# freudh/lbt

Hardware: AMD Instinct MI355X
Metric: train-step samples/sec, ResNet-20 CIFAR-10 8-bit DFP, 1/2/4/8 MI355X (higher is better)
Workload: dtype int8; 1 GPU; ResNet-20 CIFAR-10 8-bit DFXP W/A/G train step (fwd+bwd+SGD-momentum+range update); global_batch=128, per_gpu_batch=128, parallelism=dp1, hip_graph=True, executor=fused, grad_range=-6, loss_diverged=False

## Files before the change

### include/lbt_dfxp.h

```cpp
#ifndef LBT_DFXP_H
#define LBT_DFXP_H

#include <stdint.h>

#ifdef __cplusplus
extern "C" {
#endif

#define LBT_OK 0
#define LBT_EINVAL 1001

#define LBT_NSHARD 32
#define LBT_CSTRIDE 32

enum {
  LBT_OUT_I8 = 0,
  LBT_OUT_U8OFF = 1,
  LBT_OUT_I16 = 2,
  LBT_OUT_F32 = 3
};

typedef struct lbt_qdesc {
  const int32_t* exps;
  int32_t* counts;
// ... 191 lines not shown
                             lbt_qdesc qw, const int8_t* gq2, const int8_t* wd2, int32_t ksd2,
                             lbt_conv_desc d2, lbt_qdesc qg2, lbt_qdesc qw2, int32_t w4,
                             const lbt_chain_bwd_a* a, void* stream);
int lbt_conv_dgrad_chain_i8w4(const int8_t* gq, const uint8_t* wd4, int32_t ksd, lbt_conv_desc d, lbt_qdesc qg,
                              lbt_qdesc qw, const float* add_src, const lbt_chain_bwd_a* a, void* stream);
int lbt_conv_dgrad_chain_wgrad_i8(const int8_t* gq, const int8_t* wd, int32_t ksd, lbt_conv_desc d, lbt_qdesc qg,
                                  lbt_qdesc qw, const float* add_src, const lbt_chain_bwd_a* a, const int8_t* xq,
                                  int32_t x_u8off, int32_t* slab, int32_t nsplit, int32_t nshard, void* stream);
int lbt_conv_dgrad_chain_wgrad_i8w4(const int8_t* gq, const uint8_t* wd4, int32_t ksd, lbt_conv_desc d,
                                    lbt_qdesc qg, lbt_qdesc qw, const float* add_src, const lbt_chain_bwd_a* a,
                                    const int8_t* xq, int32_t x_u8off, int32_t* slab, int32_t nsplit,
                                    int32_t nshard, void* stream);

typedef struct lbt_chain_bwd_b {
  const int8_t* G; lbt_qdesc qng; const int8_t* qn_codes; lbt_qdesc qn; const float* ms;
  const int64_t* sums; int64_t n;
  float* dx; int8_t* gq; lbt_qdesc qo; int64_t* gcolsum;
  int64_t rows, inner; int32_t C;
} lbt_chain_bwd_b;
int lbt_bn_chain_bwd_b(const lbt_chain_bwd_b* a, void* stream);
int lbt_conv_stem_bwd(const lbt_chain_bwd_b* b, const int16_t* x, lbt_conv_desc d, int32_t* slab, int32_t nshard,
                      void* stream);
int lbt_bn_chain_bwd_b_pair(const lbt_chain_bwd_b* a, const lbt_chain_bwd_b* b, void* stream);

typedef struct lbt_wgrad_job {
  const int8_t* xq; int32_t x_u8off; const int8_t* gq; lbt_conv_desc d;
  int32_t* slab; int32_t nsplit, nshard;
} lbt_wgrad_job;

int lbt_conv_wgrad_many_i8(const lbt_wgrad_job* jobs, int32_t njobs, void* stream);
int lbt_conv_wgrad_many_stem_i8(const lbt_wgrad_job* jobs, int32_t njobs, const lbt_chain_bwd_b* b, const int16_t* x,
                                lbt_conv_desc d, int32_t* slab, int32_t nshard, void* stream);

typedef struct lbt_conv_bwd {
  lbt_chain_bwd_b b;
  const int8_t* wd; int32_t ksd; int32_t w4; lbt_conv_desc d; lbt_qdesc qw;
  const float* add_src;
  lbt_chain_bwd_a a;
  lbt_wgrad_job w;
} lbt_conv_bwd;
int lbt_conv_bwd_fused_i8(const lbt_conv_bwd* p, void* stream);

typedef struct lbt_conv_bwd2 {
  lbt_chain_bwd_b b1, bs;
  const int8_t* wd1; int32_t ksd1; const int8_t* wds; int32_t ksds; int32_t w4;
  lbt_conv_desc d1, ds; lbt_qdesc qw1, qws;
  lbt_chain_bwd_a a;
} lbt_conv_bwd2;
int lbt_conv_bwd2_fused_i8(const lbt_conv_bwd2* p, void* stream);

typedef struct lbt_conv_fwd {
  lbt_chain_fwd c;
  const int8_t* wf; int32_t ksf; int32_t w4; const int32_t* wcolsum; lbt_conv_desc d; lbt_qdesc qw;
  int8_t* yq; lbt_qdesc qout; int64_t* ychsum;
} lbt_conv_fwd;
int lbt_conv_fwd_fused_i8(const lbt_conv_fwd* p, void* stream);

int lbt_conv_fused_tile_rows(int32_t Cin, int64_t N, int32_t H);

int lbt_bn_bwd_a_wide(const float* g, lbt_qdesc qrg, const int8_t* R, const float* gamma_q, lbt_qdesc qng,
                      const int8_t* qn, int16_t* gout, float* dout, int64_t* sums, int64_t rows, int64_t inner,
                      int32_t C, void* stream);
int lbt_bn_bwd_b_wide(const int16_t* G, lbt_qdesc qng, const int8_t* qn, lbt_qdesc qn_q, const float* ms,
                      const int64_t* sums, int64_t n, float* dx, int64_t rows, int32_t C, void* stream);

int lbt_bn_bwd_a_wide_masked(const float* g, const float* g2, const float* y_mask, const uint8_t* y_bits,
// ... 176 lines not shown
```

### lbt_amd/_lib.py

```python
import ctypes
import os

import torch

HERE = os.path.dirname(os.path.abspath(__file__))
LIB_PATH = os.environ.get("LBT_LIBRARY") or os.path.join(HERE, "liblbt_dfxp.so")

NSHARD = 32
STEM_WG_PIXELS = 256
CSTRIDE = 32
OUT_I8, OUT_U8OFF, OUT_I16, OUT_F32 = 0, 1, 2, 3
ABI_VERSION = 22

c_void_p, c_int32, c_int64, c_uint32, c_uint64, c_float = (
    ctypes.c_void_p, ctypes.c_int32, ctypes.c_int64, ctypes.c_uint32, ctypes.c_uint64, ctypes.c_float)


class QDesc(ctypes.Structure):
    _fields_ = [("exps", c_void_p), ("counts", c_void_p), ("step", c_void_p), ("seed", c_uint64),
                ("qid", c_uint32), ("slot", c_int32), ("bits", c_int32), ("stochastic", c_int32),
                ("noise", c_void_p)]


NO_Q = QDesc()


class ConvDesc(ctypes.Structure):
    _fields_ = [(n, c_int32) for n in ("N", "H", "W", "Cin", "Cout", "KH", "KW", "SH", "SW",
                                       "PT", "PB", "PL", "PR", "Ho", "Wo")]


class BnNorm(ctypes.Structure):
    _fields_ = [("q", c_void_p), ("qn", QDesc), ("chsum", c_void_p), ("n", c_int64),
                ("eps", c_float), ("momentum", c_float), ("one_minus_momentum", c_float),
                ("ms", c_void_p), ("run_mean", c_void_p), ("run_var", c_void_p), ("frozen", c_int32),
                ("ms_in", c_int32)]


class ChainBranch(ctypes.Structure):
    _fields_ = [("nrm", BnNorm), ("xin", c_void_p), ("qr", QDesc), ("rout", c_void_p), ("gb", c_void_p)]


class ChainFwd(ctypes.Structure):
    _fields_ = [("b1", ChainBranch), ("b2", ChainBranch), ("has_b2", c_int32),
                ("res", c_void_p), ("relu", c_int32), ("y", c_void_p),
# ... 141 lines not shown
    "lbt_dfxp_counts_fold": [_P, c_int32, _P, _P],
    "lbt_dfxp_range_update_folded": [_P, _P, _P, _P, _P, c_int32, _P, _P],
    "lbt_dfxp_quantize_weight": [_P, c_int32, c_int32, c_int32, c_int32, QDesc, _P, _P, c_int32, _P, c_int32,
                                 _P, _P],
    "lbt_conv_fwd_i8": [_P, c_int32, _P, c_int32, _P, ConvDesc, QDesc, QDesc, _P, _P, QDesc, _P, _P],
    "lbt_conv_dgrad_i8": [_P, _P, c_int32, ConvDesc, QDesc, QDesc, _P, _P, _P],
    "lbt_conv_fwd_i8w4": [_P, c_int32, _P, c_int32, _P, ConvDesc, QDesc, QDesc, _P, _P, QDesc, _P, _P],
    "lbt_conv_dgrad_i8w4": [_P, _P, c_int32, ConvDesc, QDesc, QDesc, _P, _P, _P],
    "lbt_pack_int4": [_P, _P, c_int64, _P],
    "lbt_conv_fwd_igemm": [_P, c_int32, _P, c_int32, _P, ConvDesc, QDesc, QDesc, _P, _P],
    "lbt_conv_dgrad_igemm": [_P, c_int32, _P, c_int32, ConvDesc, QDesc, QDesc, _P, _P, _P],
    "lbt_conv_wgrad_igemm": [_P, _P, c_int32, ConvDesc, _P, c_int32, c_int32, _P],
    "lbt_igemm_workspace_bytes": [ConvDesc, c_int32, c_int32],
    "lbt_igemm_get_tuning": [_P],
    "lbt_igemm_set_tuning": [_P],
    "lbt_conv_fwd_igemm_q": [_P, c_int32, _P, c_int32, ConvDesc, QDesc, QDesc, _P, QDesc, _P, _P],
    "lbt_conv_fwd_igemm_ws": [_P, c_int32, _P, c_int32, _P, ConvDesc, QDesc, QDesc, _P, _P, c_int64, _P],
    "lbt_conv_dgrad_igemm_ws": [_P, c_int32, _P, c_int32, ConvDesc, QDesc, QDesc, _P, _P, _P, c_int64, _P],
    "lbt_conv_dgrad_igemm_bna": [_P, _P, c_int32, ConvDesc, QDesc, QDesc, ctypes.POINTER(DgradBna), _P, _P, c_int64,
                                 _P],
    "lbt_bn_moments": [ctypes.POINTER(BnNorm), c_int32, _P],
    "lbt_conv_dgrad_igemm_bn3": [_P, _P, c_int32, ConvDesc, QDesc, QDesc, ctypes.POINTER(DgradBn3), _P, _P, c_int64,
                                 _P],
    "lbt_conv_wgrad_igemm_store": [_P, _P, c_int32, ConvDesc, _P, c_int32, _P],
    "lbt_conv_dgrad_chain_i8w4": [_P, _P, c_int32, ConvDesc, QDesc, QDesc, _P, _P, _P],
    "lbt_conv_dgrad_chain_i8": [_P, _P, c_int32, ConvDesc, QDesc, QDesc, _P, _P, _P],
    "lbt_conv_dgrad_chain_wgrad_i8": [_P, _P, c_int32, ConvDesc, QDesc, QDesc, _P, _P, _P, c_int32, _P, c_int32,
                                      c_int32, _P],
    "lbt_conv_dgrad_chain_wgrad_i8w4": [_P, _P, c_int32, ConvDesc, QDesc, QDesc, _P, _P, _P, c_int32, _P, c_int32,
                                        c_int32, _P],
    "lbt_conv_wgrad_i8": [_P, c_int32, _P, ConvDesc, _P, c_int32, c_int32, _P],
    "lbt_conv_wgrad_many_i8": [_P, c_int32, _P],
    "lbt_conv_wgrad_many_stem_i8": [_P, c_int32, _P, _P, ConvDesc, _P, c_int32, _P],
    "lbt_conv_wgrad_reduce": [_P, c_int32, c_int32, c_int32, c_int32, _P, QDesc, QDesc, _P, c_float, _P, _P],
    "lbt_conv_fwd_generic": [_P, c_int32, _P, ConvDesc, QDesc, QDesc, _P, _P],
    "lbt_conv_dgrad_generic": [_P, _P, ConvDesc, QDesc, QDesc, _P, _P, _P],
    "lbt_conv_wgrad_generic": [_P, c_int32, _P, ConvDesc, _P, c_int32, _P],
    "lbt_conv_dgrad_generic16": [_P, _P, ConvDesc, QDesc, QDesc, _P, _P, _P],
    "lbt_conv_wgrad_generic16": [_P, c_int32, _P, ConvDesc, _P, c_int32, _P],
    "lbt_conv_wgrad_reduce64": [_P, c_int32, c_int32, c_int32, QDesc, QDesc, _P, c_float, _P, _P],
    "lbt_conv_wgrad_reduce64_many": [_P, c_int32, c_int32, _P],
    "lbt_conv_stem_fwd": [_P, _P, ConvDesc, QDesc, QDesc, _P, _P, QDesc, _P, _P],
    "lbt_conv_stem_wgrad": [_P, _P, ConvDesc, _P, c_int32, _P],
    "lbt_conv_stem_bwd": [_P, _P, ConvDesc, _P, c_int32, _P],
    "lbt_conv_bwd2_fused_i8": [_P, _P],
    "lbt_conv_fwd2_fused_i8": [_P, _P],
    "lbt_conv_wgrad_reduce_x": [_P, c_int32, c_int32, c_int32, c_int32, _P, _P, _P],
    "lbt_conv_wgrad_reduce64_x": [_P, c_int32, c_int32, c_int32, _P, _P],
    "lbt_dense_wgrad_x": [_P, _P, c_int32, c_int32, c_int32, c_int32, _P, _P],
    "lbt_bn_param_grads_x": [_P, c_int32, _P, _P, _P],
    "lbt_softmax_xent_n": [_P, _P, c_int32, c_int32, c_int32, _P, _P, _P, _P],
    "lbt_softmax_xent_wide_n": [_P, _P, c_int32, c_int32, c_int32, _P, _P, _P, _P],
    "lbt_conv_stem_wide_fwd": [_P, _P, ConvDesc, QDesc, QDesc, _P, _P],
    "lbt_stem_wide_nsplit": [ConvDesc],
    "lbt_conv_stem_wide_wgrad": [_P, c_int32, _P, c_int32, ConvDesc, _P, c_int32, _P],
    "lbt_dense_pack": [_P, c_int32, c_int32, _P, c_int32, _P, c_int32, _P],
    "lbt_flat_weight_blocks": [c_int64],
    "lbt_dfxp_quantize_weights_flat": [_P, _P, c_int32, c_int32, _P],
    "lbt_bn_bwd_a_wide_masked": [_P, _P, _P, _P, c_int32, QDesc, _P, _P, QDesc, _P, QDesc, _P, _P, _P, _P, c_int64, c_int64,
                                 c_int32, _P],
    "lbt_bn_bwd_b_wide_q": [_P, QDesc, _P, QDesc, _P, _P, c_int64, _P, QDesc, c_int64, c_int64, c_int32, _P],
    "lbt_dense_gemm": [_P, c_int32, c_int32, c_int32, _P, c_int32, c_int32, c_int32, QDesc, QDesc, _P, _P],
    "lbt_dense_wgrad": [_P, _P, c_int32, c_int32, c_int32, c_int32, QDesc, QDesc, _P, c_float, _P, _P],
    "lbt_softmax_xent_wide": [_P, _P, c_int32, c_int32, _P, _P, _P],
    "lbt_bn_chain_fwd": [_P, _P],
    "lbt_bn_chain_bwd_a": [_P, _P],
# ... 96 lines not shown
```

### lbt_amd/csrc/conv_mfma.hip

```cpp
#include "conv_epilogue.h"
#include "chain_flags.h"
#include "conv_wgrad_body.h"
#include "lds_tr.h"
#include "stem_bwd.h"

using namespace lbt;

namespace {

constexpr int kThreads = 256;

enum { MODE_FWD = 0, MODE_DGRAD = 1 };

struct GemmArgs {
  const int8_t* a;
  const int8_t* b;
  int ks;
  int nslices;
  int a_fill;
  const int32_t* colsum;
  lbt_conv_desc d;
  lbt_qdesc qa, qb;
  float* y;
  const float* add_src;
  int8_t* yq;
  lbt_qdesc qout;
  int64_t* ychsum;
  int64_t M;
  int ncol;
  lbt_chain_bwd_a chain;
};

template <int MODE, int CS, int NT, int CF, int NB, bool W4, bool DUAL = false>
__device__ __forceinline__ void conv_gemm_body(const GemmArgs& p, uint32_t bid, const GemmArgs* p2 = nullptr) {
  using G = EpiGeom<NT>;
  constexpr int NTW = G::NTW, WPM = G::WPM, MTB = G::MTB;
  __shared__ EpiShared<NT> sh;
// ... 530 lines not shown
                                             lbt_qdesc qg, lbt_qdesc qw, const float* add_src,
                                             const lbt_chain_bwd_a* a, const int8_t* xq, int32_t x_u8off,
                                             int32_t* slab, int32_t nsplit, int32_t nshard, void* stream) {
  return dgrad_chain_wgrad<false>(gq, wd, ksd, d, qg, qw, add_src, a, xq, x_u8off, slab, nsplit, nshard, stream);
}
extern "C" int lbt_conv_dgrad_chain_wgrad_i8w4(const int8_t* gq, const uint8_t* wd4, int32_t ksd, lbt_conv_desc d,
                                               lbt_qdesc qg, lbt_qdesc qw, const float* add_src,
                                               const lbt_chain_bwd_a* a, const int8_t* xq, int32_t x_u8off,
                                               int32_t* slab, int32_t nsplit, int32_t nshard, void* stream) {
  if (qw.bits > 4) return LBT_EINVAL;
  return dgrad_chain_wgrad<true>(gq, (const int8_t*)wd4, ksd, d, qg, qw, add_src, a, xq, x_u8off, slab, nsplit,
                                 nshard, stream);
}

extern "C" int lbt_conv_wgrad_i8(const int8_t* xq, int32_t x_u8off, const int8_t* gq, lbt_conv_desc d,
                                    int32_t* slab, int32_t nsplit, int32_t nshard, void* stream) {
  WgradArgs wa;
  uint32_t blocks = 0;
  const int e = wgrad_setup(xq, x_u8off, gq, d, slab, nsplit, nshard, wa, blocks);
  if (e) return e;
  hipStream_t st = (hipStream_t)stream;
  switch (d.Cin / 16) {
    case 1: hipLaunchKernelGGL(conv_wgrad_kernel<1>, dim3(blocks), dim3(kThreads), 0, st, wa); break;
    case 2: hipLaunchKernelGGL(conv_wgrad_kernel<2>, dim3(blocks), dim3(kThreads), 0, st, wa); break;
    case 4: hipLaunchKernelGGL(conv_wgrad_kernel<4>, dim3(blocks), dim3(kThreads), 0, st, wa); break;
    case 8: hipLaunchKernelGGL(conv_wgrad_kernel<8>, dim3(blocks), dim3(kThreads), 0, st, wa); break;
    default: return LBT_EINVAL;
  }
  return (int)hipGetLastError();
}

namespace {
constexpr int kMaxWJobs = 24;
#ifndef LBT_WGM_OCC
#define LBT_WGM_OCC 4
#endif
#ifndef LBT_WGM_BUFS
#define LBT_WGM_BUFS 2
#endif
#ifndef LBT_WGX
#define LBT_WGX 0
#endif
constexpr int kWgmBufs = LBT_WGM_BUFS;
constexpr int kFW = 8;
constexpr int kHaloMax = 3;
struct WgradMany {
  WgradArgs j[kMaxWJobs];
  uint32_t start[kMaxWJobs + 1];
  int32_t fast[kMaxWJobs];
  int n;
};
union WgradManyShared {
  WgradShared<1, kFW> s1;
  WgradShared<2, kFW> s2;
  int8_t stage[kFW][5 * 1024];
  int red[kFW / 2][9 * 256];
};

bool wgrad_s1_ok(const lbt_conv_desc& d, int nsplit) {
  if (d.KH != 3 || d.KW != 3 || d.SH != 1 || d.SW != 1 || d.PT != 1 || d.PB != 1 || d.PL != 1 || d.PR != 1 ||
      d.Ho != d.H || d.Wo != d.W || d.W > 64 || 64 % d.W || d.H % (64 / d.W) ||
      (64 / d.W + 2) * (d.W + 2) > 64 * kHaloMax)
    return false;
  const int64_t chunks = (int64_t)d.N * d.H * d.W / 64;
  return nsplit > 0 && chunks % nsplit == 0;
}

LBT_DEV v4i tr_frag_at(const int8_t* img, int oa, int ob) {
  typedef __attribute__((address_space(3))) v2i lds_v2i;
  const v2i lo = __builtin_amdgcn_ds_read_tr8_b64_v2i32((lds_v2i*)(img + oa));
  const v2i hi = __builtin_amdgcn_ds_read_tr8_b64_v2i32((lds_v2i*)(img + ob));
  return v4i{lo.x, lo.y, hi.x, hi.y};
}

__device__ __forceinline__ void wgrad_s1_body(const WgradArgs& wa, uint32_t bid, WgradManyShared& sm) {
  const lbt_conv_desc& d = wa.d;
  const int H = d.H, W = d.W, Cin = d.Cin, Cout = d.Cout;
  const int ncs = Cin >> 4, ncos = Cout >> 4, nsplit = wa.nsplit;
  const int total = nsplit * ncs * ncos;
  const int xchunk = (total + 7) >> 3;
  const int u = (int)(bid & 7) * xchunk + (int)(bid >> 3);
  if (u >= total) return;
  const int split = u / (ncs * ncos), urem = u - split * (ncs * ncos);
  const int cis = urem / ncos, cos = urem - cis * ncos;
  const int lane = threadIdx.x & 63, wave = wave_id();
  const int j = lane & 15, kg = lane >> 4;
  const int RB = 64 / W, Wp = W + 2, nhalo = (RB + 2) * Wp;
  const int64_t cps = (int64_t)d.N * H * W / 64 / nsplit;
  const int64_t c0 = (int64_t)split * cps;
  const int nmine = cps > wave ? (int)((cps - wave + kFW - 1) / kFW) : 0;
  const int HW = H * W;
  const int fill = wa.x_fill;
  int8_t* st = sm.stage[wave];
  int8_t* gs = st + 4096;
  const int pa = 16 * kg + (j >> 1), pb = pa + 8;
  const int oxa = ((pa / W) * Wp + pa % W) * 16 + 8 * (j & 1);
  const int oxb = ((pb / W) * Wp + pb % W) * 16 + 8 * (j & 1);
  const int oga = pa * 16 + 8 * (j & 1), ogb = pb * 16 + 8 * (j & 1);
  int hoff[kHaloMax];
  uint32_t hin = 0, htop = 0, hbot = 0;
#pragma unroll
  for (int i = 0; i < kHaloMax; ++i) {
    const int t = lane + 64 * i;
    const int hy = t / Wp, hx = t - hy * Wp;
    hoff[i] = ((hy - 1) * W + hx - 1) * Cin;
    hin |= (uint32_t)(t < nhalo && hx >= 1 && hx <= W) << i;
    htop |= (uint32_t)(hy == 0) << i;
    hbot |= (uint32_t)(hy == RB + 1) << i;
  }

  struct Buf {
    v4i x[kHaloMax], g;
    uint32_t valid;
  };
  auto load = [&](Buf& b, int64_t c) {
    const int64_t p0 = c * 64;
    const int n = (int)(p0 / HW), row0 = (int)(p0 - (int64_t)n * HW) / W;
    const int8_t* xim = wa.xq + (p0 * Cin + cis * 16);
    b.valid = hin & ~(row0 == 0 ? htop : 0u) & ~(row0 + RB == H ? hbot : 0u);
#pragma unroll
    for (int i = 0; i < kHaloMax; ++i)
      b.x[i] = *reinterpret_cast<const v4i*>(xim + ((b.valid >> i) & 1 ? hoff[i] : 0));
    b.g = *reinterpret_cast<const v4i*>(wa.gq + (p0 + lane) * Cout + cos * 16);
  };
  v4i acc[9];
#pragma unroll
  for (int t = 0; t < 9; ++t) acc[t] = v4i{0, 0, 0, 0};
  auto cidx = [&](int s) { return c0 + wave + (int64_t)(s < nmine ? s : nmine - 1) * kFW; };
  auto step = [&](Buf& b, int s) {
    if constexpr (!(LBT_WGX & 2)) {
#pragma unroll
      for (int i = 0; i < kHaloMax; ++i) {
        const int t = lane + 64 * i;
        const v4i v = (b.valid >> i) & 1 ? b.x[i] : v4i{fill, fill, fill, fill};
        if (t < nhalo) *reinterpret_cast<v4i*>(st + t * 16) = v;
      }
      *reinterpret_cast<v4i*>(gs + lane * 16) = s < nmine ? b.g : v4i{0, 0, 0, 0};
    }
    asm volatile("" ::: "memory");
    if constexpr (!(LBT_WGX & 1)) load(b, cidx(s + kWgmBufs));
    const v4i bfrag = (LBT_WGX & 4) ? b.g : tr_frag_at(gs, oga, ogb);
#pragma unroll
    for (int t = 0; t < 9; ++t) {
      const int toff = ((t / 3) * Wp + t % 3) * 16;
      const v4i afrag = (LBT_WGX & 4) ? b.x[t % kHaloMax] : tr_frag_at(st, oxa + toff, oxb + toff);
      if constexpr (LBT_WGX & 8)
        acc[t] = acc[t] + afrag + bfrag;
      else
        acc[t] = __builtin_amdgcn_mfma_i32_16x16x64_i8(afrag, bfrag, acc[t], 0, 0, 0);
    }
    asm volatile("" ::: "memory");
  };
  LBT_TS(0);
  if (nmine > 0) {
    Buf bf[kWgmBufs];
#pragma unroll
    for (int k = 0; k < kWgmBufs; ++k) load(bf[k], cidx(k));
    for (int s = 0; s < nmine; s += kWgmBufs) {
#pragma unroll
      for (int k = 0; k < kWgmBufs; ++k) step(bf[k], s + k);
    }
  }
  LBT_TS(1);
  __syncthreads();
  constexpr int kHalf = kFW / 2;
  if (wave < kHalf) {
#pragma unroll
    for (int t = 0; t < 9; ++t) *reinterpret_cast<v4i*>(&sm.red[wave][(t * 64 + lane) * 4]) = acc[t];
  }
  __syncthreads();
  if (wave >= kHalf) {
#pragma unroll
    for (int t = 0; t < 9; ++t) {
      v4i* q = reinterpret_cast<v4i*>(&sm.red[wave - kHalf][(t * 64 + lane) * 4]);
      *q = *q + acc[t];
    }
  }
  __syncthreads();
  LBT_TS(2);
  int32_t* dst = wa.slab + (int64_t)(split % wa.nshard) * 9 * Cin * Cout + (int64_t)cis * 16 * Cout + cos * 16;
  for (int i = threadIdx.x; i < 9 * 256; i += kFW * 64) {
    int v = 0;
#pragma unroll
    for (int w = 0; w < kHalf; ++w) v += sm.red[w][i];
    const int t = i >> 8, l = (i >> 2) & 63, ii = i & 3;
    const int ci = 4 * (l >> 4) + ii, co = l & 15;
    if (v) LBT_GADD(&dst[((int64_t)t * Cin + ci) * Cout + co], v);
  }
  LBT_TS(3);
}

LBT_DEV void wgrad_many_block(const WgradMany& m, uint32_t b, WgradManyShared& sm) {
  int j = 0;
#pragma unroll 1
  while (j + 1 < m.n && b >= m.start[j + 1]) ++j;
  const WgradArgs& wa = m.j[j];
  const uint32_t rb = b - m.start[j];
#ifdef LBT_TRACE
  if (threadIdx.x == 0 && lbt_trace_buf) lbt_trace_buf[(size_t)blockIdx.x * 8 + 6] = (unsigned long long)(j + 1);
#endif
  if (m.fast[j]) {
    wgrad_s1_body(wa, rb, sm);
    return;
  }
  switch (wa.d.Cin >> 4) {
    case 1: conv_wgrad_body<1, kFW>(wa, rb, sm.s1); break;
    default: conv_wgrad_body<2, kFW>(wa, rb, sm.s2); break;
  }
}

__global__ __launch_bounds__(kFW * 64, LBT_WGM_OCC) void conv_wgrad_many_kernel(const WgradMany m) {
  __shared__ __attribute__((aligned(16))) WgradManyShared sm;
  wgrad_many_block(m, blockIdx.x, sm);
}

union WgradManyStemShared {
  WgradManyShared w;
  StemBwdShared<2> s;
};
static_assert(kFW * 64 == 2 * 256, "two stem row blocks per workgroup of the batched launch");
__global__ __launch_bounds__(kFW * 64, LBT_WGM_OCC) void conv_wgrad_many_stem_kernel(const WgradMany m,
                                                                                    const StemBwdArgs st,
                                                                                    uint32_t pairs, int stem_first) {
  __shared__ __attribute__((aligned(16))) WgradManyStemShared sm;
  const uint32_t b = blockIdx.x, nw = m.start[m.n];
  if (stem_first ? b < pairs : b >= nw) {
    stem_bwd_body<2>(st, stem_first ? b : b - nw, sm.s);
    return;
  }
  wgrad_many_block(m, stem_first ? b - pairs : b, sm.w);
}
static_assert(sizeof(WgradMany) + sizeof(StemBwdArgs) + 8 <= 4096, "kernel arguments");
static_assert(sizeof(WgradMany) <= 4096, "kernel arguments");

int wgrad_many_setup(const lbt_wgrad_job& w, WgradArgs& wa, uint32_t& blocks, int32_t& fast) {
  if (!w.slab || !w.xq || !w.gq) return LBT_EINVAL;
  const int e = wgrad_setup(w.xq, w.x_u8off, w.gq, w.d, w.slab, w.nsplit, w.nshard, wa, blocks);
  if (e) return e;
  fast = wgrad_s1_ok(w.d, w.nsplit) ? 1 : 0;
  if (fast) {
    const int64_t units = (int64_t)w.nsplit * (w.d.Cin / 16) * (w.d.Cout / 16);
    blocks = (uint32_t)((units + 7) / 8 * 8);
  } else if (w.d.Cin != 16 && w.d.Cin != 32) {
    return LBT_EINVAL;
  }
  return 0;
}
}

extern "C" int lbt_conv_wgrad_many_i8(const lbt_wgrad_job* jobs, int32_t njobs, void* stream) {
  if (njobs < 0 || (njobs > 0 && !jobs)) return LBT_EINVAL;
  for (int i = 0; i < njobs; ++i) {
    WgradArgs wa;
    uint32_t blocks = 0;
    int32_t fast = 0;
    const int e = wgrad_many_setup(jobs[i], wa, blocks, fast);
    if (e) return e;
  }
  for (int base = 0; base < njobs; base += kMaxWJobs) {
    WgradMany m{};
    const int n = njobs - base < kMaxWJobs ? njobs - base : kMaxWJobs;
    uint64_t total = 0;
    for (int i = 0; i < n; ++i) {
      uint32_t blocks = 0;
      wgrad_many_setup(jobs[base + i], m.j[i], blocks, m.fast[i]);
      m.start[i] = (uint32_t)total;
      total += blocks;
    }
    if (total >= 0x7fffffffull) return LBT_EINVAL;
    m.start[n] = (uint32_t)total;
    m.n = n;
    hipLaunchKernelGGL(conv_wgrad_many_kernel, dim3((unsigned)total), dim3(kFW * 64), 0, (hipStream_t)stream, m);
    const int rc = (int)hipGetLastError();
    if (rc) return rc;
  }
  return 0;
}

extern "C" int lbt_conv_stem_bwd(const lbt_chain_bwd_b* b, const int16_t* x, lbt_conv_desc d, int32_t* slab,
                                 int32_t nshard, void* stream);
// ... 64 lines not shown
```

### lbt_amd/csrc/quantize.hip

```cpp
#include "dfxp_device.h"

using namespace lbt;

namespace {

constexpr int kThreads = 256;

__global__ __launch_bounds__(kThreads) void quantize_rows_kernel(
    const float* __restrict__ x, void* __restrict__ out, int out_kind, int64_t rows, int64_t inner,
    int rpt, lbt_qdesc q, int64_t* __restrict__ chsum, int C) {
  extern __shared__ long long sh_sum[];
  __shared__ int sh_cnt[2 * kThreads / 64];
  const QState s = qstate(q);
  const int64_t groups = inner >> 2;
  const int64_t g = (int64_t)blockIdx.x * kThreads + threadIdx.x;
  const int64_t r0 = (int64_t)blockIdx.y * rpt;
  if (chsum) {
    for (int i = threadIdx.x; i < 2 * C; i += kThreads) sh_sum[i] = 0;
    __syncthreads();
  }
  int ov1 = 0, ov2 = 0;
  int s1[4] = {0, 0, 0, 0}, s2[4] = {0, 0, 0, 0};
  if (g < groups) {
    Noise4 n = {{0.f, 0.f, 0.f, 0.f}};
// ... 231 lines not shown
  if (sgd_blocks + rblocks >= ((int64_t)1 << 31)) return LBT_EINVAL;
  hipLaunchKernelGGL(step_update_kernel, dim3((unsigned)(sgd_blocks + rblocks)), dim3(256), 0, (hipStream_t)stream, w, a,
                     g, n, lr, mu, gscale, (int)sgd_blocks, exps, counts, bits, target, nelem, nslots, step, vec);
  return (int)hipGetLastError();
}

extern "C" int lbt_dfxp_counts_fold(int32_t* counts, int32_t nslots, float* folded, void* stream) {
  if (nslots <= 0) return LBT_OK;
  hipLaunchKernelGGL(counts_fold_kernel, dim3((nslots + 3) / 4), dim3(256), 0, (hipStream_t)stream, counts, nslots,
                     folded);
  return (int)hipGetLastError();
}

extern "C" int lbt_dfxp_range_update_folded(int32_t* exps, const float* folded, const int32_t* bits,
                                            const float* target, const float* nelem, int32_t nslots,
                                            uint64_t* step, void* stream) {
  const int blocks = nslots > 0 ? (nslots + 255) / 256 : 1;
  hipLaunchKernelGGL(range_update_folded_kernel, dim3(blocks), dim3(256), 0, (hipStream_t)stream, exps, folded,
                     bits, target, nelem, nslots, step);
  return (int)hipGetLastError();
}

extern "C" int lbt_dfxp_quantize_weight(const float* w, int32_t KH, int32_t KW, int32_t Cin, int32_t Cout,
                                        lbt_qdesc q, int8_t* w_hwio, int8_t* wf, int32_t ksf, int8_t* wd,
                                        int32_t ksd, int32_t* colsum, void* stream) {
  if (q.bits < 1 || q.bits > 8) return LBT_EINVAL;
  if (wf && ksf * 16 < KH * KW * ((Cin + 15) / 16) * 16) return LBT_EINVAL;
  if (wd && ksd * 16 < KH * KW * ((Cout + 15) / 16) * 16) return LBT_EINVAL;
  hipLaunchKernelGGL(quantize_weight_kernel, dim3(Cout), dim3(kThreads), 0, (hipStream_t)stream, w, KH, KW, Cin,
                     Cout, q, w_hwio, wf, ksf, wd, ksd, colsum);
  return (int)hipGetLastError();
}

extern "C" int lbt_abi_version(void) { return 22; }
```

### lbt_amd/dfxp/ops.py

```python
import ctypes
import math
import os

import torch

from .. import _lib
from .._lib import NSHARD, OUT_F32, OUT_I8, OUT_I16, OUT_U8OFF, ConvDesc, QDesc, call, ptr, stream

NO_Q = _lib.NO_Q

PROFILE = None


class _Timed:
    def __init__(self, kernel, nbytes):
        self.kernel, self.nbytes = kernel, nbytes

    def __enter__(self):
        if PROFILE is not None:
            self.e0 = torch.cuda.Event(enable_timing=True)
            self.e1 = torch.cuda.Event(enable_timing=True)
            self.e0.record()
        return self

# ... 121 lines not shown


def _conv_dgrad_i8(gq, wd, ksd, d, qg, qw, dx, add_src):
    call("lbt_conv_dgrad_i8", ptr(gq), ptr(wd), int(ksd), d, qg, qw, ptr(dx), ptr(add_src), stream())


def pack_int4(src, dst):
    call("lbt_pack_int4", ptr(src), ptr(dst), src.numel(), stream())


def conv_fwd_i8w4(xq, x_u8off, wf4, ksf, wcolsum, d, qx, qw, y):
    M = d.N * d.Ho * d.Wo
    with _Timed("conv_fwd_i8w4", xq.numel() + wf4.numel() + M * d.Cout * 4):
        call("lbt_conv_fwd_i8w4", ptr(xq), int(x_u8off), ptr(wf4), int(ksf), ptr(wcolsum), d, qx, qw, ptr(y), None,
             NO_Q, None, stream())


def conv_dgrad_i8w4(gq, wd4, ksd, d, qg, qw, dx):
    with _Timed("conv_dgrad_i8w4", gq.numel() + wd4.numel() + dx.numel() * 4):
        call("lbt_conv_dgrad_i8w4", ptr(gq), ptr(wd4), int(ksd), d, qg, qw, ptr(dx), None, stream())


def wgrad_nsplit(d, generic=False):
    P = d.N * d.Ho * d.Wo
    taps = d.KH * d.KW
    if generic:
        lo = -(-P // 8192)
        return max(lo, min(256, -(-P // (8 if P <= 4096 else 32))))
    lo = -(-P // 65536)
    want = max(1, -(-512 // (taps * (d.Cout // 16))))
    return max(lo, min(want, max(1, P // 512)))


def wgrad_s1_ok(d):
    return (d.KH == 3 and d.KW == 3 and d.SH == 1 and d.SW == 1 and d.PT == 1 and d.PB == 1 and d.PL == 1
            and d.PR == 1 and d.Ho == d.H and d.Wo == d.W and d.W <= 64 and 64 % d.W == 0
            and d.H % (64 // d.W) == 0 and (64 // d.W + 2) * (d.W + 2) <= 192)


WGRAD_CPW = int(os.environ.get("LBT_WGRAD_CPW", "8"))
WGRAD_MIN_UNITS = int(os.environ.get("LBT_WGRAD_MIN_UNITS", "32"))
WGRAD_UNITS = int(os.environ.get("LBT_WGRAD_UNITS", "64"))


def wgrad_nsplit_batched(d, chunks_per_wave=None):
    P = d.N * d.Ho * d.Wo
    if wgrad_s1_ok(d):
        chunks = P // 64
        ns = max(1, chunks // (8 * (chunks_per_wave or WGRAD_CPW)))
        if chunks_per_wave is None:
            units = (d.Cin // 16) * (d.Cout // 16)
            while ns * units < WGRAD_MIN_UNITS and 2 * ns * 8 <= chunks:
                ns *= 2
        while chunks % ns:
            ns -= 1
        return ns
    lo = -(-P // 65536)
    return max(lo, min(max(1, WGRAD_UNITS // (d.KH * d.KW * (d.Cout // 16))), max(1, P // 512)))


def wgrad_nshard(d, nsplit):
    P = d.N * d.Ho * d.Wo
    per = -(-P // nsplit)
    return -(-nsplit // max(1, 65536 // per))


def wgrad_slab(cache, key, d, ctx, batched=False):
    ns = wgrad_nsplit_batched(d) if batched else wgrad_nsplit(d)
    nh = wgrad_nshard(d, ns)
    n = nh * d.KH * d.KW * d.Cin * d.Cout
    slab = cache.sums(key, (n + 1) // 2, ctx).view(torch.int32)[:n].view(nh, d.KH * d.KW * d.Cin, d.Cout)
    return ns, nh, slab


def conv_wgrad_i8(xq, x_u8off, gq, d, slab, nsplit, nshard):
    with _Timed("conv_wgrad_i8", xq.numel() + gq.numel() + nshard * d.KH * d.KW * d.Cin * d.Cout * 4):
        _conv_wgrad_i8(xq, x_u8off, gq, d, slab, nsplit, nshard)


def _conv_wgrad_i8(xq, x_u8off, gq, d, slab, nsplit, nshard):
    call("lbt_conv_wgrad_i8", ptr(xq), int(x_u8off), ptr(gq), d, ptr(slab), int(nsplit), int(nshard), stream())


_XSINK = None


def set_exchange_sink(gbase=None, n=0, xbuf=None, loss_off=0, world=1):
    global _XSINK
    _XSINK = None if gbase is None else dict(gbase=gbase.data_ptr(), n=int(n), xbuf=xbuf.data_ptr(),
                                             loss=xbuf.data_ptr() + 8 * int(loss_off), world=int(world))

# ... 559 lines not shown
```

Baseline: 315,200 samples/s.

## Rewrite batched wgrad fast path with async LDS loads and multi-Cout tiles

```diff
diff --git a/include/lbt_dfxp.h b/include/lbt_dfxp.h
--- a/include/lbt_dfxp.h
+++ b/include/lbt_dfxp.h
@@ -247,6 +247,10 @@
 int lbt_conv_wgrad_many_stem_i8(const lbt_wgrad_job* jobs, int32_t njobs, const lbt_chain_bwd_b* b, const int16_t* x,
                                 lbt_conv_desc d, int32_t* slab, int32_t nshard, void* stream);
 
+int lbt_conv_wgrad_many_nsplit(lbt_conv_desc d, int32_t chunks_per_wave, int32_t tap_units);
+int lbt_conv_wgrad_many_blocks(lbt_conv_desc d, int32_t nsplit);
+int lbt_conv_wgrad_many_slots(void);
+
 typedef struct lbt_conv_bwd {
   lbt_chain_bwd_b b;
   const int8_t* wd; int32_t ksd; int32_t w4; lbt_conv_desc d; lbt_qdesc qw;
diff --git a/lbt_amd/_lib.py b/lbt_amd/_lib.py
--- a/lbt_amd/_lib.py
+++ b/lbt_amd/_lib.py
@@ -10,7 +10,7 @@
 STEM_WG_PIXELS = 256
 CSTRIDE = 32
 OUT_I8, OUT_U8OFF, OUT_I16, OUT_F32 = 0, 1, 2, 3
-ABI_VERSION = 22
+ABI_VERSION = 23
 
 c_void_p, c_int32, c_int64, c_uint32, c_uint64, c_float = (
     ctypes.c_void_p, ctypes.c_int32, ctypes.c_int64, ctypes.c_uint32, ctypes.c_uint64, ctypes.c_float)
@@ -218,6 +218,9 @@
     "lbt_conv_wgrad_i8": [_P, c_int32, _P, ConvDesc, _P, c_int32, c_int32, _P],
     "lbt_conv_wgrad_many_i8": [_P, c_int32, _P],
     "lbt_conv_wgrad_many_stem_i8": [_P, c_int32, _P, _P, ConvDesc, _P, c_int32, _P],
+    "lbt_conv_wgrad_many_nsplit": [ConvDesc, c_int32, c_int32],
+    "lbt_conv_wgrad_many_blocks": [ConvDesc, c_int32],
+    "lbt_conv_wgrad_many_slots": [],
     "lbt_conv_wgrad_reduce": [_P, c_int32, c_int32, c_int32, c_int32, _P, QDesc, QDesc, _P, c_float, _P, _P],
     "lbt_conv_fwd_generic": [_P, c_int32, _P, ConvDesc, QDesc, QDesc, _P, _P],
     "lbt_conv_dgrad_generic": [_P, _P, ConvDesc, QDesc, QDesc, _P, _P, _P],
diff --git a/lbt_amd/csrc/conv_mfma.hip b/lbt_amd/csrc/conv_mfma.hip
--- a/lbt_amd/csrc/conv_mfma.hip
+++ b/lbt_amd/csrc/conv_mfma.hip
@@ -3,6 +3,9 @@
 #include "conv_wgrad_body.h"
 #include "lds_tr.h"
 #include "stem_bwd.h"
+
+#include <algorithm>
+#include <utility>
 
 using namespace lbt;
 
@@ -599,17 +602,13 @@
 
 namespace {
 constexpr int kMaxWJobs = 24;
-#ifndef LBT_WGM_OCC
-#define LBT_WGM_OCC 4
-#endif
-#ifndef LBT_WGM_BUFS
-#define LBT_WGM_BUFS 2
-#endif
-#ifndef LBT_WGX
-#define LBT_WGX 0
-#endif
-constexpr int kWgmBufs = LBT_WGM_BUFS;
+constexpr int kWgmOcc = 4;
+constexpr int kWgmBufs = 2;
+constexpr int kWgmBuf = 4096;
 constexpr int kFW = 8;
+constexpr int kWgmCpw = 16;
+constexpr int kWgmMinUnits = 8;
+constexpr int kWgmTapUnits = 16;
 constexpr int kHaloMax = 3;
 struct WgradMany {
   WgradArgs j[kMaxWJobs];
@@ -620,139 +619,206 @@
 union WgradManyShared {
   WgradShared<1, kFW> s1;
   WgradShared<2, kFW> s2;
-  int8_t stage[kFW][5 * 1024];
+  int8_t stage[kFW][kWgmBufs * kWgmBuf];
   int red[kFW / 2][9 * 256];
 };
 
-bool wgrad_s1_ok(const lbt_conv_desc& d, int nsplit) {
-  if (d.KH != 3 || d.KW != 3 || d.SH != 1 || d.SW != 1 || d.PT != 1 || d.PB != 1 || d.PL != 1 || d.PR != 1 ||
-      d.Ho != d.H || d.Wo != d.W || d.W > 64 || 64 % d.W || d.H % (64 / d.W) ||
-      (64 / d.W + 2) * (d.W + 2) > 64 * kHaloMax)
-    return false;
-  const int64_t chunks = (int64_t)d.N * d.H * d.W / 64;
-  return nsplit > 0 && chunks % nsplit == 0;
-}
-
-LBT_DEV v4i tr_frag_at(const int8_t* img, int oa, int ob) {
-  typedef __attribute__((address_space(3))) v2i lds_v2i;
-  const v2i lo = __builtin_amdgcn_ds_read_tr8_b64_v2i32((lds_v2i*)(img + oa));
-  const v2i hi = __builtin_amdgcn_ds_read_tr8_b64_v2i32((lds_v2i*)(img + ob));
+int wgrad_s1_variant(const lbt_conv_desc& d, int nsplit) {
+  if (d.KH != 3 || d.KW != 3 || d.SH != d.SW || (d.SH != 1 && d.SH != 2) || d.PT < 0 || d.PT > 1 || d.PL < 0 ||
+      d.PL > 1 || d.Wo <= 0 || d.Wo > 64 || 64 % d.Wo || d.Ho % (64 / d.Wo))
+    return 0;
+  if (d.SH == 1 && (d.PT != 1 || d.PB != 1 || d.PL != 1 || d.PR != 1 || d.Ho != d.H || d.Wo != d.W)) return 0;
+  const int64_t chunks = (int64_t)d.N * d.Ho * d.Wo / 64;
+  if (nsplit <= 0 || chunks % nsplit) return 0;
+  if ((chunks / nsplit + kFW - 1) / kFW * 64 > 65536) return 0;
+  const int nhalo = ((64 / d.Wo - 1) * d.SH + 3) * ((d.Wo - 1) * d.SH + 3), nh = (nhalo + 63) / 64;
+  const bool co2 = (d.Cout / 16) % 2 == 0;
+  if (d.SH == 2) return (co2 && nh <= 5) ? 4 : 0;
+  if (nh > kHaloMax) return 0;
+  if (nh == 3) return 1;
+  return co2 ? 3 : 2;
+}
+int wgrad_s1_nco(int variant) { return variant >= 3 ? 2 : 1; }
+
+static __device__ __attribute__((aligned(16))) uint32_t kWgFill80[4] = {0x80808080u, 0x80808080u, 0x80808080u,
+                                                                        0x80808080u};
+typedef __attribute__((address_space(3))) void* wg_lds_vptr;
+template <int N>
+LBT_DEV void wg_vm_wait() {
+  static_assert(N >= 0 && N < 64, "vmcnt");
+  asm volatile("s_waitcnt vmcnt(%0)" ::"n"(N) : "memory");
+}
+template <int OFF>
+LBT_DEV v4i wg_tr_frag(uint32_t a, uint32_t b) {
+  v2i lo, hi;
+  asm volatile("ds_read_b64_tr_b8 %0, %1 offset:%2" : "=v"(lo) : "v"(a), "n"(OFF) : "memory");
+  asm volatile("ds_read_b64_tr_b8 %0, %1 offset:%2" : "=v"(hi) : "v"(b), "n"(OFF) : "memory");
   return v4i{lo.x, lo.y, hi.x, hi.y};
 }
-
+LBT_DEV void wg_tr_wait(v4i& a) { asm volatile("s_waitcnt lgkmcnt(0)" : "+v"(a)::"memory"); }
+LBT_DEV void wg_tr_wait(v4i& a, v4i& b) { asm volatile("s_waitcnt lgkmcnt(0)" : "+v"(a), "+v"(b)::"memory"); }
+LBT_DEV void wg_tr_wait(v4i& a, v4i& b, v4i& c) {
+  asm volatile("s_waitcnt lgkmcnt(0)" : "+v"(a), "+v"(b), "+v"(c)::"memory");
+}
+
+template <int I>
+using wg_int = std::integral_constant<int, I>;
+template <class F, int... I>
+LBT_DEV void wg_static_for(F&& f, std::integer_sequence<int, I...>) {
+  (f(wg_int<I>{}), ...);
+}
+
+template <int NCO, int NH, int S = 1, int NB = kWgmBufs>
 __device__ __forceinline__ void wgrad_s1_body(const WgradArgs& wa, uint32_t bid, WgradManyShared& sm) {
+  constexpr int kBuf = kWgmBufs * kWgmBuf / NB;
+  static_assert((NH + NCO) * 1024 <= kBuf && (NB == 1 || NB == kWgmBufs), "one ring buffer");
   const lbt_conv_desc& d = wa.d;
-  const int H = d.H, W = d.W, Cin = d.Cin, Cout = d.Cout;
-  const int ncs = Cin >> 4, ncos = Cout >> 4, nsplit = wa.nsplit;
-  const int total = nsplit * ncs * ncos;
+  const int H = d.H, W = d.W, Wo = d.Wo, Cin = d.Cin, Cout = d.Cout;
+  const int ncs = Cin >> 4, ncog = (Cout >> 4) / NCO, nsplit = wa.nsplit;
+  const int total = nsplit * ncs * ncog;
   const int xchunk = (total + 7) >> 3;
   const int u = (int)(bid & 7) * xchunk + (int)(bid >> 3);
   if (u >= total) return;
-  const int split = u / (ncs * ncos), urem = u - split * (ncs * ncos);
-  const int cis = urem / ncos, cos = urem - cis * ncos;
+  const int split = u / (ncs * ncog), urem = u - split * (ncs * ncog);
+  const int cis = urem / ncog, cog = urem - cis * ncog;
   const int lane = threadIdx.x & 63, wave = wave_id();
   const int j = lane & 15, kg = lane >> 4;
-  const int RB = 64 / W, Wp = W + 2, nhalo = (RB + 2) * Wp;
-  const int64_t cps = (int64_t)d.N * H * W / 64 / nsplit;
-  const int64_t c0 = (int64_t)split * cps;
-  const int nmine = cps > wave ? (int)((cps - wave + kFW - 1) / kFW) : 0;
-  const int HW = H * W;
-  const int fill = wa.x_fill;
-  int8_t* st = sm.stage[wave];
-  int8_t* gs = st + 4096;
+  const int RB = 64 / Wo, WR = (RB - 1) * S + 3, Wp = (Wo - 1) * S + 3, nhalo = WR * Wp;
+  const int bpi = d.Ho / RB;
+  const int cps = (int)((int64_t)d.N * bpi / nsplit);
+  const int c0 = split * cps;
+  const int nmine = cps > wave ? (cps - wave + kFW - 1) / kFW : 0;
+  const int8_t* xfill = wa.x_fill ? reinterpret_cast<const int8_t*>(kWgFill80) : reinterpret_cast<const int8_t*>(zi());
+  const int8_t* zero = reinterpret_cast<const int8_t*>(zi());
+  int8_t* region = sm.stage[wave];
+  typedef __attribute__((address_space(3))) int8_t wg_lds_i8;
+  const uint32_t rbase = (uint32_t)(uintptr_t)(wg_lds_i8*)region;
   const int pa = 16 * kg + (j >> 1), pb = pa + 8;
-  const int oxa = ((pa / W) * Wp + pa % W) * 16 + 8 * (j & 1);
-  const int oxb = ((pb / W) * Wp + pb % W) * 16 + 8 * (j & 1);
-  const int oga = pa * 16 + 8 * (j & 1), ogb = pb * 16 + 8 * (j & 1);
-  int hoff[kHaloMax];
+  uint32_t xa[3], xb[3];
+#pragma unroll
+  for (int r = 0; r < 3; ++r) {
+    xa[r] = rbase + (uint32_t)((((pa / Wo) * S + r) * Wp + (pa % Wo) * S) * 16 + 8 * (j & 1));
+    xb[r] = rbase + (uint32_t)((((pb / Wo) * S + r) * Wp + (pb % Wo) * S) * 16 + 8 * (j & 1));
+  }
+  const uint32_t ga = rbase + (uint32_t)(NH * 1024 + pa * 16 * NCO + 8 * (j & 1));
+  const uint32_t gb = rbase + (uint32_t)(NH * 1024 + pb * 16 * NCO + 8 * (j & 1));
+  const int hbot0 = H - (d.Ho - RB) * S + d.PT;
+  int hoff[NH], goff[NCO];
   uint32_t hin = 0, htop = 0, hbot = 0;
 #pragma unroll
-  for (int i = 0; i < kHaloMax; ++i) {
+  for (int i = 0; i < NH; ++i) {
     const int t = lane + 64 * i;
     const int hy = t / Wp, hx = t - hy * Wp;
-    hoff[i] = ((hy - 1) * W + hx - 1) * Cin;
-    hin |= (uint32_t)(t < nhalo && hx >= 1 && hx <= W) << i;
-    htop |= (uint32_t)(hy == 0) << i;
-    hbot |= (uint32_t)(hy == RB + 1) << i;
-  }
-
-  struct Buf {
-    v4i x[kHaloMax], g;
-    uint32_t valid;
-  };
-  auto load = [&](Buf& b, int64_t c) {
-    const int64_t p0 = c * 64;
-    const int n = (int)(p0 / HW), row0 = (int)(p0 - (int64_t)n * HW) / W;
-    const int8_t* xim = wa.xq + (p0 * Cin + cis * 16);
-    b.valid = hin & ~(row0 == 0 ? htop : 0u) & ~(row0 + RB == H ? hbot : 0u);
-#pragma unroll
-    for (int i = 0; i < kHaloMax; ++i)
-      b.x[i] = *reinterpret_cast<const v4i*>(xim + ((b.valid >> i) & 1 ? hoff[i] : 0));
-    b.g = *reinterpret_cast<const v4i*>(wa.gq + (p0 + lane) * Cout + cos * 16);
-  };
-  v4i acc[9];
-#pragma unroll
-  for (int t = 0; t < 9; ++t) acc[t] = v4i{0, 0, 0, 0};
-  auto cidx = [&](int s) { return c0 + wave + (int64_t)(s < nmine ? s : nmine - 1) * kFW; };
-  auto step = [&](Buf& b, int s) {
-    if constexpr (!(LBT_WGX & 2)) {
-#pragma unroll
-      for (int i = 0; i < kHaloMax; ++i) {
-        const int t = lane + 64 * i;
-        const v4i v = (b.valid >> i) & 1 ? b.x[i] : v4i{fill, fill, fill, fill};
-        if (t < nhalo) *reinterpret_cast<v4i*>(st + t * 16) = v;
+    hoff[i] = ((hy - d.PT) * W + hx - d.PL) * Cin;
+    hin |= (uint32_t)(t < nhalo && hx >= d.PL && hx < W + d.PL) << i;
+    htop |= (uint32_t)(hy < d.PT) << i;
+    hbot |= (uint32_t)(hy >= hbot0) << i;
+  }
+#pragma unroll
+  for (int c = 0; c < NCO; ++c) {
+    const int q = lane + 64 * c;
+    goff[c] = (q / NCO) * Cout + (cog * NCO + q % NCO) * 16;
+  }
+  v4i acc[9][NCO];
+#pragma unroll
+  for (int t = 0; t < 9; ++t)
+#pragma unroll
+    for (int c = 0; c < NCO; ++c) acc[t][c] = v4i{0, 0, 0, 0};
+
+  constexpr int kDma = NH + NCO;
+  int ic = c0 + wave, in = ic / bpi, im = ic - in * bpi;
+  const int instep = kFW / bpi, imstep = kFW - instep * bpi;
+  auto issue = [&](int k, int s) {
+    const int64_t p0 = (int64_t)ic * 64, x0 = ((int64_t)in * H + im * (RB * S)) * W;
+    const int8_t* xim = wa.xq + (x0 * Cin + cis * 16);
+    const uint32_t valid = hin & ~(im == 0 ? htop : 0u) & ~(im == bpi - 1 ? hbot : 0u);
+    int8_t* b = region + k * kBuf;
+#pragma unroll
+    for (int i = 0; i < NH; ++i)
+      __builtin_amdgcn_global_load_lds((valid >> i) & 1 ? xim + hoff[i] : xfill, (wg_lds_vptr)(b + i * 1024), 16, 0, 0);
+    const int8_t* gim = wa.gq + p0 * Cout;
+#pragma unroll
+    for (int c = 0; c < NCO; ++c)
+      __builtin_amdgcn_global_load_lds(s < nmine ? gim + goff[c] : zero, (wg_lds_vptr)(b + (NH + c) * 1024), 16, 0, 0);
+    if (s + 1 < nmine) {
+      ic += kFW;
+      in += instep;
+      im += imstep;
+      if (im >= bpi) {
+        im -= bpi;
+        ++in;
       }
-      *reinterpret_cast<v4i*>(gs + lane * 16) = s < nmine ? b.g : v4i{0, 0, 0, 0};
-    }
-    asm volatile("" ::: "memory");
-    if constexpr (!(LBT_WGX & 1)) load(b, cidx(s + kWgmBufs));
-    const v4i bfrag = (LBT_WGX & 4) ? b.g : tr_frag_at(gs, oga, ogb);
-#pragma unroll
-    for (int t = 0; t < 9; ++t) {
-      const int toff = ((t / 3) * Wp + t % 3) * 16;
-      const v4i afrag = (LBT_WGX & 4) ? b.x[t % kHaloMax] : tr_frag_at(st, oxa + toff, oxb + toff);
-      if constexpr (LBT_WGX & 8)
-        acc[t] = acc[t] + afrag + bfrag;
-      else
-        acc[t] = __builtin_amdgcn_mfma_i32_16x16x64_i8(afrag, bfrag, acc[t], 0, 0, 0);
-    }
-    asm volatile("" ::: "memory");
+    }
   };
   LBT_TS(0);
   if (nmine > 0) {
-    Buf bf[kWgmBufs];
-#pragma unroll
-    for (int k = 0; k < kWgmBufs; ++k) load(bf[k], cidx(k));
-    for (int s = 0; s < nmine; s += kWgmBufs) {
-#pragma unroll
-      for (int k = 0; k < kWgmBufs; ++k) step(bf[k], s + k);
-    }
+    if constexpr (NB > 1) {
+#pragma unroll
+      for (int k = 0; k < NB; ++k) issue(k, k);
+    }
+    for (int s = 0; s < nmine; s += NB) {
+      wg_static_for(
+          [&](auto K) {
+            constexpr int k = decltype(K)::value, kb = k * kBuf;
+            if constexpr (NB == 1) issue(0, s);
+            wg_vm_wait<(NB - 1) * kDma>();
+            v4i bf[NCO];
+            wg_static_for([&](auto C) { bf[decltype(C)::value] = wg_tr_frag<kb + decltype(C)::value * 16>(ga, gb); },
+                          std::make_integer_sequence<int, NCO>{});
+            v4i af = wg_tr_frag<kb>(xa[0], xb[0]);
+            if constexpr (NCO == 2)
+              wg_tr_wait(bf[0], bf[1], af);
+            else
+              wg_tr_wait(bf[0], af);
+            wg_static_for(
+                [&](auto T) {
+                  constexpr int t = decltype(T)::value;
+                  v4i an = af;
+                  if constexpr (t < 8) an = wg_tr_frag<kb + ((t + 1) % 3) * 16>(xa[(t + 1) / 3], xb[(t + 1) / 3]);
+#pragma unroll
+                  for (int c = 0; c < NCO; ++c)
+                    acc[t][c] = __builtin_amdgcn_mfma_i32_16x16x64_i8(af, bf[c], acc[t][c], 0, 0, 0);
+                  if constexpr (t < 8) {
+                    wg_tr_wait(an);
+                    af = an;
+                  }
+                },
+                std::make_integer_sequence<int, 9>{});
+            if constexpr (NB > 1) issue(k, s + k + NB);
+          },
+          std::make_integer_sequence<int, NB>{});
+    }
+    wg_vm_wait<0>();
   }
   LBT_TS(1);
-  __syncthreads();
   constexpr int kHalf = kFW / 2;
-  if (wave < kHalf) {
-#pragma unroll
-    for (int t = 0; t < 9; ++t) *reinterpret_cast<v4i*>(&sm.red[wave][(t * 64 + lane) * 4]) = acc[t];
-  }
-  __syncthreads();
-  if (wave >= kHalf) {
-#pragma unroll
-    for (int t = 0; t < 9; ++t) {
-      v4i* q = reinterpret_cast<v4i*>(&sm.red[wave - kHalf][(t * 64 + lane) * 4]);
-      *q = *q + acc[t];
-    }
-  }
-  __syncthreads();
-  LBT_TS(2);
-  int32_t* dst = wa.slab + (int64_t)(split % wa.nshard) * 9 * Cin * Cout + (int64_t)cis * 16 * Cout + cos * 16;
-  for (int i = threadIdx.x; i < 9 * 256; i += kFW * 64) {
-    int v = 0;
-#pragma unroll
-    for (int w = 0; w < kHalf; ++w) v += sm.red[w][i];
-    const int t = i >> 8, l = (i >> 2) & 63, ii = i & 3;
-    const int ci = 4 * (l >> 4) + ii, co = l & 15;
-    if (v) LBT_GADD(&dst[((int64_t)t * Cin + ci) * Cout + co], v);
+#pragma unroll
+  for (int c = 0; c < NCO; ++c) {
+    __syncthreads();
+    if (wave < kHalf) {
+#pragma unroll
+      for (int t = 0; t < 9; ++t) *reinterpret_cast<v4i*>(&sm.red[wave][(t * 64 + lane) * 4]) = acc[t][c];
+    }
+    __syncthreads();
+    if (wave >= kHalf) {
+#pragma unroll
+      for (int t = 0; t < 9; ++t) {
+        v4i* q = reinterpret_cast<v4i*>(&sm.red[wave - kHalf][(t * 64 + lane) * 4]);
+        *q = *q + acc[t][c];
+      }
+    }
+    __syncthreads();
+    if (c == 0) LBT_TS(2);
+    int32_t* dst = wa.slab + (int64_t)(split % wa.nshard) * 9 * Cin * Cout + (int64_t)cis * 16 * Cout +
+                   (cog * NCO + c) * 16;
+    for (int i = threadIdx.x; i < 9 * 256; i += kFW * 64) {
+      int v = 0;
+#pragma unroll
+      for (int w = 0; w < kHalf; ++w) v += sm.red[w][i];
+      const int t = i >> 8, l = (i >> 2) & 63, ii = i & 3;
+      const int ci = 4 * (l >> 4) + ii, co = l & 15;
+      if (v) LBT_GADD(&dst[((int64_t)t * Cin + ci) * Cout + co], v);
+    }
   }
   LBT_TS(3);
 }
@@ -766,9 +832,12 @@
 #ifdef LBT_TRACE
   if (threadIdx.x == 0 && lbt_trace_buf) lbt_trace_buf[(size_t)blockIdx.x * 8 + 6] = (unsigned long long)(j + 1);
 #endif
-  if (m.fast[j]) {
-    wgrad_s1_body(wa, rb, sm);
-    return;
+  switch (m.fast[j]) {
+    case 1: wgrad_s1_body<1, 3>(wa, rb, sm); return;
+    case 2: wgrad_s1_body<1, 2>(wa, rb, sm); return;
+    case 3: wgrad_s1_body<2, 2>(wa, rb, sm); return;
+    case 4: wgrad_s1_body<2, 5, 2, 1>(wa, rb, sm); return;
+    default: break;
   }
   switch (wa.d.Cin >> 4) {
     case 1: conv_wgrad_body<1, kFW>(wa, rb, sm.s1); break;
@@ -776,7 +845,7 @@
   }
 }
 
-__global__ __launch_bounds__(kFW * 64, LBT_WGM_OCC) void conv_wgrad_many_kernel(const WgradMany m) {
+__global__ __launch_bounds__(kFW * 64, kWgmOcc) void conv_wgrad_many_kernel(const WgradMany m) {
   __shared__ __attribute__((aligned(16))) WgradManyShared sm;
   wgrad_many_block(m, blockIdx.x, sm);
 }
@@ -786,7 +855,7 @@
   StemBwdShared<2> s;
 };
 static_assert(kFW * 64 == 2 * 256, "two stem row blocks per workgroup of the batched launch");
-__global__ __launch_bounds__(kFW * 64, LBT_WGM_OCC) void conv_wgrad_many_stem_kernel(const WgradMany m,
+__global__ __launch_bounds__(kFW * 64, kWgmOcc) void conv_wgrad_many_stem_kernel(const WgradMany m,
                                                                                     const StemBwdArgs st,
                                                                                     uint32_t pairs, int stem_first) {
   __shared__ __attribute__((aligned(16))) WgradManyStemShared sm;
@@ -804,15 +873,55 @@
   if (!w.slab || !w.xq || !w.gq) return LBT_EINVAL;
   const int e = wgrad_setup(w.xq, w.x_u8off, w.gq, w.d, w.slab, w.nsplit, w.nshard, wa, blocks);
   if (e) return e;
-  fast = wgrad_s1_ok(w.d, w.nsplit) ? 1 : 0;
+  fast = wgrad_s1_variant(w.d, w.nsplit);
   if (fast) {
-    const int64_t units = (int64_t)w.nsplit * (w.d.Cin / 16) * (w.d.Cout / 16);
+    const int64_t units = (int64_t)w.nsplit * (w.d.Cin / 16) * (w.d.Cout / 16 / wgrad_s1_nco(fast));
     blocks = (uint32_t)((units + 7) / 8 * 8);
   } else if (w.d.Cin != 16 && w.d.Cin != 32) {
     return LBT_EINVAL;
   }
   return 0;
 }
+}
+
+extern "C" int lbt_conv_wgrad_many_slots(void) {
+  static const int cus = [] {
+    int dev = 0, n = 0;
+    if (hipGetDevice(&dev) != hipSuccess ||
+        hipDeviceGetAttribute(&n, hipDeviceAttributeMultiprocessorCount, dev) != hipSuccess || n <= 0)
+      n = 256;
+    return n;
+  }();
+  return cus * (kWgmOcc * 4 / kFW);
+}
+
+extern "C" int lbt_conv_wgrad_many_blocks(lbt_conv_desc d, int32_t nsplit) {
+  if (!desc_ok(d) || d.Cin % 16 || d.Cout % 16 || nsplit <= 0) return -LBT_EINVAL;
+  const int v = wgrad_s1_variant(d, nsplit);
+  if (!v && d.Cin != 16 && d.Cin != 32) return -LBT_EINVAL;
+  const int64_t units = v ? (int64_t)nsplit * (d.Cin / 16) * (d.Cout / 16 / wgrad_s1_nco(v))
+                          : (int64_t)nsplit * d.KH * d.KW * (d.Cout / 16);
+  return units < ((int64_t)1 << 30) ? (int)((units + 7) / 8 * 8) : -LBT_EINVAL;
+}
+
+extern "C" int lbt_conv_wgrad_many_nsplit(lbt_conv_desc d, int32_t chunks_per_wave, int32_t tap_units) {
+  if (!desc_ok(d) || d.Cin % 16 || d.Cout % 16) return -LBT_EINVAL;
+  const int64_t P = (int64_t)d.N * d.Ho * d.Wo;
+  const int v = wgrad_s1_variant(d, 1);
+  if (!v) {
+    const int64_t lo = (P + 65535) / 65536, taps = (int64_t)d.KH * d.KW * (d.Cout / 16);
+    const int64_t want = std::max<int64_t>(1, (tap_units > 0 ? tap_units : kWgmTapUnits) / taps);
+    return (int)std::max(lo, std::min(want, std::max<int64_t>(1, P / 512)));
+  }
+  const int64_t chunks = P / 64, units = (int64_t)(d.Cin / 16) * (d.Cout / 16 / wgrad_s1_nco(v));
+  const int cpw = chunks_per_wave > 0 ? chunks_per_wave : kWgmCpw;
+  int64_t ns = std::max<int64_t>(1, chunks / ((int64_t)kFW * cpw));
+  if (chunks_per_wave <= 0) {
+    while (ns * units < kWgmMinUnits && 2 * ns * kFW <= chunks) ns *= 2;
+  }
+  ns = std::max(ns, (chunks + kFW * 1024 - 1) / (kFW * 1024));
+  while (chunks % ns) --ns;
+  return (int)ns;
 }
 
 extern "C" int lbt_conv_wgrad_many_i8(const lbt_wgrad_job* jobs, int32_t njobs, void* stream) {
diff --git a/lbt_amd/csrc/quantize.hip b/lbt_amd/csrc/quantize.hip
--- a/lbt_amd/csrc/quantize.hip
+++ b/lbt_amd/csrc/quantize.hip
@@ -287,4 +287,4 @@
   return (int)hipGetLastError();
 }
 
-extern "C" int lbt_abi_version(void) { return 22; }
+extern "C" int lbt_abi_version(void) { return 23; }
diff --git a/lbt_amd/dfxp/ops.py b/lbt_amd/dfxp/ops.py
--- a/lbt_amd/dfxp/ops.py
+++ b/lbt_amd/dfxp/ops.py
@@ -177,31 +177,22 @@
     return max(lo, min(want, max(1, P // 512)))
 
 
-def wgrad_s1_ok(d):
-    return (d.KH == 3 and d.KW == 3 and d.SH == 1 and d.SW == 1 and d.PT == 1 and d.PB == 1 and d.PL == 1
-            and d.PR == 1 and d.Ho == d.H and d.Wo == d.W and d.W <= 64 and 64 % d.W == 0
-            and d.H % (64 // d.W) == 0 and (64 // d.W + 2) * (d.W + 2) <= 192)
-
-
-WGRAD_CPW = int(os.environ.get("LBT_WGRAD_CPW", "8"))
-WGRAD_MIN_UNITS = int(os.environ.get("LBT_WGRAD_MIN_UNITS", "32"))
-WGRAD_UNITS = int(os.environ.get("LBT_WGRAD_UNITS", "64"))
+WGRAD_CPW = int(os.environ.get("LBT_WGRAD_CPW", "0"))
+WGRAD_UNITS = int(os.environ.get("LBT_WGRAD_UNITS", "0"))
 
 
 def wgrad_nsplit_batched(d, chunks_per_wave=None):
-    P = d.N * d.Ho * d.Wo
-    if wgrad_s1_ok(d):
-        chunks = P // 64
-        ns = max(1, chunks // (8 * (chunks_per_wave or WGRAD_CPW)))
-        if chunks_per_wave is None:
-            units = (d.Cin // 16) * (d.Cout // 16)
-            while ns * units < WGRAD_MIN_UNITS and 2 * ns * 8 <= chunks:
-                ns *= 2
-        while chunks % ns:
-            ns -= 1
-        return ns
-    lo = -(-P // 65536)
-    return max(lo, min(max(1, WGRAD_UNITS // (d.KH * d.KW * (d.Cout // 16))), max(1, P // 512)))
+    ns = _lib.load().lbt_conv_wgrad_many_nsplit(d, int(chunks_per_wave or WGRAD_CPW), WGRAD_UNITS)
+    if ns <= 0:
+        raise _lib.LbtError("lbt_conv_wgrad_many_nsplit = %d" % ns)
+    return ns
+
+
+def wgrad_many_blocks(d, nsplit):
+    nb = _lib.load().lbt_conv_wgrad_many_blocks(d, int(nsplit))
+    if nb <= 0:
+        raise _lib.LbtError("lbt_conv_wgrad_many_blocks = %d" % nb)
+    return nb
 
 
 def wgrad_nshard(d, nsplit):
```

Result: no change. 323,300 samples/s (median of 6 runs) (+2.5%).
